# thu-ml/stochastic_gcn

Hardware: AMD Instinct MI355X
Metric: training edges/s (SpMM) (higher is better)
Workload: dtype f32

## Files before the change

### profiles/epoch_profile.py

```python
#!/usr/bin/env python
import glob
import os
import sqlite3
import sys

ROOT = os.path.dirname(os.path.dirname(os.path.abspath(__file__)))
sys.path.insert(0, ROOT)


def run(epochs):
    import torch
    import bench
    from stochastic_gcn_amd import _ffi
    for kv in os.environ.get("SGCN_TUNE", "").split():
        k, v = kv.split("=")
        _ffi.tune(k, int(v))
    from stochastic_gcn_amd import synthetic
    from stochastic_gcn_amd.flags import FLAGS
    over = {}
    for kv in os.environ.get("SGCN_FLAGS", "").split():
        k, v = kv.split("=")
        over[k] = type(getattr(FLAGS, k))(int(v)) if isinstance(getattr(FLAGS, k), (bool, int)) else float(v)
    if over:
        orig = FLAGS.update
        FLAGS.update = lambda **kw: (orig(**kw), orig(**over))[0]
    data = synthetic.reddit_like(seed=1, with_features=False)
    te = bench.train_epoch_leg(data, torch.device("cuda:0"), epochs=epochs)
    print(te, file=sys.stderr)


def summarize(src, steps):
    f = glob.glob(os.path.join(src, "**", "*results.db"), recursive=True)
    t = sqlite3.connect(f[0])
    rows = list(t.execute("select name,total_calls,total_duration,average,percentage from top_kernels"))
    tot = sum(r[2] for r in rows)
    print("== rocprofv3 --kernel-trace --stats of profiles/epoch_profile.py: %d training steps "
          "(batch 512, CVD+PP, S-Reddit), all kernels incl. set-up" % steps)
    print("GPU-busy total %.1f ms = %.3f ms per step (upper bound: includes the one-off PP SpMM and set-up kernels)"
          % (tot / 1e3, tot / 1e3 / steps))
    print("%-92s %8s %10s %12s %10s %6s" % ("kernel", "calls", "calls/step", "total_ms", "avg_us", "pct"))
    for r in rows[:40]:
        print("%-92s %8d %10.2f %12.1f %10.2f %6.2f" % (r[0][:92], r[1], r[1] / steps, r[2] / 1e3, r[3], r[4]))


if __name__ == "__main__" and not (len(sys.argv) > 1 and sys.argv[1] in ("--gaps", "--timeline", "--stepgaps")):
    if len(sys.argv) > 1 and sys.argv[1] == "--summarize":
        summarize(sys.argv[2], int(sys.argv[3]))
    else:
        run(int(sys.argv[1]) if len(sys.argv) > 1 else 3)


def gaps(src):
    f = glob.glob(os.path.join(src, "**", "*results.db"), recursive=True)
    t = sqlite3.connect(f[0])
    tabs = [r[0] for r in t.execute("select name from sqlite_master where type in ('table','view')")]
    view = "kernels" if "kernels" in tabs else None
    if view is None:
        print("tables:", tabs)
        return
    cols = [r[1] for r in t.execute("pragma table_info(%s)" % view)]
    rows = list(t.execute("select name, start, end from %s order by start" % view))
    import numpy as np
    st = np.array([r[1] for r in rows], dtype=np.int64)
    en = np.array([r[2] for r in rows], dtype=np.int64)
    names = [r[0] for r in rows]
    lo = len(rows) * 2 // 3
    gap = (st[lo + 1:] - en[lo:-1]) / 1e3
    dur = (en[lo:] - st[lo:]) / 1e3
    span = (en[-1] - st[lo]) / 1e3
    print("steady-state window: %d kernels over %.1f ms: busy %.1f ms (%.1f %%), idle between kernels %.1f ms"
          % (len(dur), span / 1e3, dur.sum() / 1e3, 100 * dur.sum() / span, gap.sum() / 1e3))
    print("gap between consecutive kernels: median %.2f us, mean %.2f us, p90 %.2f us, share of gaps > 4 us: %.1f %%"
          % (np.median(gap), gap.mean(), np.percentile(gap, 90), 100 * (gap > 4).mean()))
    adam = [i for i in range(lo, len(rows)) if "adam_" in names[i]]
    if len(adam) > 2:
        per = np.diff(st[adam]) / 1e3
        print("step period (adam to adam): median %.1f us; kernels per step %.1f"
              % (np.median(per), (adam[-1] - adam[0]) / (len(adam) - 1)))
    qcol = "queue_id" if "queue_id" in cols else ("stream_id" if "stream_id" in cols else None)
    if qcol and len(adam) > 2:
        qs = [r[0] for r in t.execute("select %s from %s order by start" % (qcol, view))]
        a, b = adam[0], adam[-1]
        nsteps = len(adam) - 1
        per_q = {}
        for i in range(a, b):
            k = per_q.setdefault(qs[i], [0, 0.0])
            k[0] += 1
            k[1] += (en[i] - st[i]) / 1e3
        for q, (cnt, us) in sorted(per_q.items(), key=lambda kv: -kv[1][1]):
            print("queue %s: %.1f kernels and %.1f us of kernel time per step" % (q, cnt / nsteps, us / nsteps))


if __name__ == "__main__" and len(sys.argv) > 1 and sys.argv[1] == "--gaps":
    gaps(sys.argv[2])


def timeline(src, n=70):
    f = glob.glob(os.path.join(src, "**", "*results.db"), recursive=True)
    t = sqlite3.connect(f[0])
    cols = [r[1] for r in t.execute("pragma table_info(kernels)")]
    qcol = "queue_id" if "queue_id" in cols else ("stream_id" if "stream_id" in cols else None)
    rows = list(t.execute("select name, start, end%s from kernels order by start" % ((", " + qcol) if qcol else "")))
    adam = [i for i, r in enumerate(rows) if "adam_" in r[0]]
    a, b = adam[len(adam) // 2], adam[len(adam) // 2 + 1]
    t0 = rows[a][2]
    print("columns:", cols)
    for r in rows[a:b + 1][:n]:
        print("%9.2f us  +%7.2f us  q=%s  %s" % ((r[1] - t0) / 1e3, (r[2] - r[1]) / 1e3, r[3] if qcol else "-", r[0][:70]))


if __name__ == "__main__" and len(sys.argv) > 1 and sys.argv[1] == "--timeline":
    timeline(sys.argv[2])


def stepgaps(src):
    import numpy as np
    f = glob.glob(os.path.join(src, "**", "*results.db"), recursive=True)
    t = sqlite3.connect(f[0])
    rows = list(t.execute("select name, start, end from kernels order by start"))
    adam = [i for i, r in enumerate(rows) if "adam_" in r[0]]
    adam = adam[len(adam) // 3:]
    lens = np.diff(adam)
    usual = int(np.bincount(lens).argmax())
    steps = [a for a, n in zip(adam[:-1], lens) if n == usual]
    gap = np.array([[rows[a + j + 1][1] - rows[a + j][2] for j in range(usual)] for a in steps]) / 1e3
    dur = np.array([[rows[a + j + 1][2] - rows[a + j + 1][1] for j in range(usual)] for a in steps]) / 1e3
    print("%d steady-state steps of %d kernels: idle in front of each kernel / its duration (median us; p90 of the idle)"
          % (len(steps), usual))
    for j in range(usual):
        print("  idle %6.2f (p90 %6.2f)  run %6.2f  %s" % (np.median(gap[:, j]), np.percentile(gap[:, j], 90),
                                                            np.median(dur[:, j]), rows[steps[0] + j + 1][0][:60]))
    print("  per step: idle %.1f us + kernels %.1f us" % (np.median(gap.sum(1)), np.median(dur.sum(1))))
    st = np.array([rows[a][1] for a in adam], dtype=np.int64)
    per = np.diff(st) / 1e3
    per = per[per < 2000]
    busy = np.array([sum(rows[i][2] - rows[i][1] for i in range(a + 1, b + 1)) for a, b in zip(adam[:-1], adam[1:])]) / 1e3
    busy = busy[:len(np.diff(st))][np.diff(st) / 1e3 < 2000]
    slow = [(int(i), round(float(p), 1)) for i, p in enumerate(np.diff(st) / 1e3) if 160 < p < 2000]
    print("  periods over 160 us (step index in the window, us):", slow[:40])
    print("  all %d steps: period mean %.1f / median %.1f / p90 %.1f / max %.1f us; kernel time mean %.1f / p90 %.1f us"
          % (len(per), per.mean(), np.median(per), np.percentile(per, 90), per.max(), busy.mean(), np.percentile(busy, 90)))


if __name__ == "__main__" and len(sys.argv) > 1 and sys.argv[1] == "--stepgaps":
    stepgaps(sys.argv[2])
```

### stochastic_gcn_amd/csrc/sgcn_agg.hip

```cpp
#include "sgcn_dev.h"
#include <type_traits>

namespace sgcn {

int group_lanes(int nvec);

template <class HT>
struct AggArgsT {
    const int32_t* a_rowptr; const int32_t* a_col; const float* a_val;
    const int32_t* f_rowptr; const int32_t* f_col; const float* f_val;
    const sgcn_seg_t* seg; int64_t nseg; int64_t nsegblk;
    const float* h; const float* mu; int64_t ldx;
    const HT* H; int64_t ldh;
    const int32_t* ifield; const int32_t* ffield; const float* s;
    float* out_h; float* out_mu; int64_t ldo;
    int32_t d, nvec, cvd, off, concat;
    float* ws; int64_t ldw;
    int32_t pchunks;
    float* accP_out; const float* accP_in;
};


template <int VW>
__device__ __forceinline__ void store_masked(float* p, typename Vec<VW>::type v, int left) {
    if (left >= VW) vstore<VW>(p, v);
    else vstore_head<VW>(p, v, left);
}

template <int G, int VW, class HT>
__device__ __forceinline__ void agg_apart(const AggArgsT<HT>& a, int row, int vi, int lig, bool act,
                                          typename Vec<VW>::type& acc1, typename Vec<VW>::type& acc2) {
    typedef typename Vec<VW>::type VT;
    acc1 = vzero<VW>(); acc2 = vzero<VW>();
    const int start = uniform_i<G>(a.a_rowptr[row]), end = uniform_i<G>(a.a_rowptr[row + 1]);
    const int64_t voff = (int64_t)vi * VW;
    for (int p0 = start; p0 < end; p0 += G) {
        const int n = min(G, end - p0);
        int mycol = 0, myhist = 0;
        float myval = 0.f;
        if (lig < n) {
            mycol = a.a_col[p0 + lig];
            myval = a.a_val[p0 + lig];
            myhist = a.ifield[mycol];
        }
        for (int j = 0; j < n; j++) {
            const int c = bcast_i<G>(mycol, j);
            const int hr = bcast_i<G>(myhist, j);
            const float v = bcast_f<G>(myval, j);
            if (!act) continue;
            const VT hb = hload<VW>(a.H + (int64_t)hr * a.ldh + voff);
            const VT xv = vload<VW>(a.h + (int64_t)c * a.ldx + voff);
            if constexpr (VW == 1 && !std::is_same<HT, float>::value) {
                if (a.cvd) {
                    const float mv = a.mu[(int64_t)c * a.ldx + voff];
                    acc1 = __builtin_fmaf(v, mv - hb, acc1);
                    acc2 = __builtin_fmaf(v, xv - mv, acc2);
                } else {
                    acc1 = __builtin_fmaf(v, xv, acc1);
                    acc2 = __builtin_fmaf(v, hb, acc2);
                }
            } else if (a.cvd) {
                const VT mv = vload<VW>(a.mu + (int64_t)c * a.ldx + voff);
                acc1 += v * (mv - hb);
                acc2 += v * (xv - mv);
            } else {
                acc1 += v * xv;
                acc2 += v * hb;
            }
        }
    }
}

template <int VW, class HT>
__device__ __forceinline__ void agg_epilogue(const AggArgsT<HT>& a, int row, int vi, bool act, typename Vec<VW>::type accP,
                                             typename Vec<VW>::type acc1, typename Vec<VW>::type acc2) {
    typedef typename Vec<VW>::type VT;
    if (!act) return;
    const int64_t voff = (int64_t)vi * VW;
    const int left = a.d - vi * VW;
    float* oh = a.out_h + (int64_t)row * a.ldo;
    if (a.cvd) {
        float* om = a.out_mu + (int64_t)row * a.ldo;
        const VT mu_nbr = acc1 + accP;
        const VT h_nbr = acc2 * a.s[row] + mu_nbr;
        store_masked<VW>(oh + a.off + voff, h_nbr, left);
        store_masked<VW>(om + a.off + voff, mu_nbr, left);
        if (a.concat) {
            store_masked<VW>(oh + voff, vload<VW>(a.h + (int64_t)row * a.ldx + voff), left);
            store_masked<VW>(om + voff, vload<VW>(a.mu + (int64_t)row * a.ldx + voff), left);
        }
    } else {
        const VT out = (acc1 - acc2) + accP;
        store_masked<VW>(oh + a.off + voff, out, left);
        if (a.concat) store_masked<VW>(oh + voff, vload<VW>(a.h + (int64_t)row * a.ldx + voff), left);
    }
}

template <int G, int VW, class HT>
__device__ __forceinline__ void agg_finish(const AggArgsT<HT>& a, int row, int vi, int lig, bool act,
                                           typename Vec<VW>::type accP) {
    typename Vec<VW>::type acc1, acc2;
    agg_apart<G, VW>(a, row, vi, lig, act, acc1, acc2);
    agg_epilogue<VW>(a, row, vi, act, accP, acc1, acc2);
}

static int p_chunks(int32_t d, const void* Hbar, int64_t ldh, const float* ws) {
    const int vw = pick_vw(d, {Hbar, ws}, {ldh, ((int64_t)d + 3) / 4 * 4});
    return kBlock / group_lanes((d + vw - 1) / vw) - 1;
}

constexpr int agg_max_chunks(int G, int VW) { return (kBlock / G) * (4 / VW) - 1 < 31 ? (kBlock / G) * (4 / VW) - 1 : 31; }

template <int G, int VW, int U, class HT>
__global__ __launch_bounds__(kBlock) void agg_row_kernel(AggArgsT<HT> a) {
    typedef typename Vec<VW>::type VT;
    constexpr int NG = kBlock / G, NP = NG - 1;
    constexpr int NC = agg_max_chunks(G, VW);
    __shared__ float part[NC + 2][G * VW];
    const int lig = threadIdx.x & (G - 1), gq = threadIdx.x / G;
    const int slab = (int)(blockIdx.x / a.nseg);
    const int64_t s = blockIdx.x % a.nseg;
    int row, start, end, slot;
    if (a.seg) {
        const sgcn_seg_t sg = a.seg[s];
        row = sg.row; start = sg.start; end = sg.end; slot = sg.slot;
    } else {
        row = (int)s; start = a.f_rowptr[s]; end = a.f_rowptr[s + 1]; slot = -1;
    }
    row = uniform_i<G>(row); start = uniform_i<G>(start);
    end = uniform_i<G>(end); slot = uniform_i<G>(slot);
    const int vi = slab * G + lig;
    const bool act = vi < a.nvec;
    const bool finish_here = slot < 0 && !a.accP_out;
    const HT* Hl = a.H + (int64_t)vi * VW;

    const int nc = a.pchunks;
    if (gq < NP) {
        const int chunk = (end - start + nc - 1) / nc;
        for (int ck = gq; ck < nc; ck += NP) {
            const int gs = start + ck * chunk, ge = min(end, gs + chunk);
            VT accP = vzero<VW>();
            for (int p0 = gs; p0 < ge; p0 += G) {
                const int n = min(G, ge - p0);
                int myrow = 0;
                float myval = 0.f;
                if (lig < n) {
                    myrow = a.ffield[a.f_col[p0 + lig]];
                    myval = a.f_val[p0 + lig];
                }
                hpin<HT, VW>(myrow); hpin<HT, VW>(myval);
                for (int j = 0; j < n; j += U) {
                    typename HRaw<HT, VW>::type b[U];
                    float v[U];
#pragma unroll
                    for (int u = 0; u < U; u++) {
                        const bool in = j + u < n;
                        const int c = bcast_i<G>(myrow, in ? j + u : 0);
                        v[u] = in ? bcast_f<G>(myval, j + u) : 0.f;
                        b[u] = (act && in) ? hraw<VW>(Hl + (int64_t)c * a.ldh) : hraw_zero<HT, VW>();
                    }
#pragma unroll
                    for (int u = 0; u < U; u++) { hpin<HT, VW>(b[u]); accP += v[u] * hwiden<VW>(b[u]); }
                }
            }
            vstore<VW>(&part[ck][lig * VW], accP);
        }
    } else if (finish_here) {
        VT acc1, acc2;
        agg_apart<G, VW>(a, row, vi, lig, act, acc1, acc2);
        vstore<VW>(&part[NC][lig * VW], acc1);
        vstore<VW>(&part[NC + 1][lig * VW], acc2);
    }
    __syncthreads();
    if (gq != 0) return;
    VT accP = vload<VW>(&part[0][lig * VW]);
    if (nc == NP) {
#pragma unroll
        for (int q = 1; q < NP; q++) accP += vload<VW>(&part[q][lig * VW]);
    } else {
        for (int q = 1; q < nc; q++) accP += vload<VW>(&part[q][lig * VW]);
    }
    if (slot >= 0) { if (act) vstore<VW>(a.ws + (int64_t)slot * a.ldw + (int64_t)vi * VW, accP); }
    else if (a.accP_out) { if (act) vstore<VW>(a.accP_out + (int64_t)row * a.ldw + (int64_t)vi * VW, accP); }
    else agg_epilogue<VW>(a, row, vi, act, accP, vload<VW>(&part[NC][lig * VW]), vload<VW>(&part[NC + 1][lig * VW]));
}

template <int G, int VW, class HT>
__global__ __launch_bounds__(kBlock) void agg_fix_kernel(AggArgsT<HT> a, const sgcn_fix_t* fix, int64_t nfix) {
    typedef typename Vec<VW>::type VT;
    constexpr int GPB = kBlock / G;
    const int lig = threadIdx.x & (G - 1);
    const int64_t nfblk = (nfix + GPB - 1) / GPB;
    const int slab = (int)(blockIdx.x / nfblk);
    const int64_t f = (blockIdx.x % nfblk) * GPB + threadIdx.x / G;
    if (f >= nfix) return;
    const sgcn_fix_t fx = fix[f];
    const int vi = slab * G + lig;
    const bool act = vi < a.nvec;
    VT accP = vzero<VW>();
    if (act) {
        const float* w = a.ws + (int64_t)fx.first_slot * a.ldw + (int64_t)vi * VW;
        for (int q = 0; q < fx.nslots; q++) accP += vload<VW>(w + (int64_t)q * a.ldw);
    }
    if (a.accP_out) { if (act) vstore<VW>(a.accP_out + (int64_t)fx.row * a.ldw + (int64_t)vi * VW, accP); }
    else agg_finish<G, VW>(a, uniform_i<G>(fx.row), vi, lig, act, accP);
}

template <int G, int VW, class HT>
__global__ __launch_bounds__(kBlock) void agg_post_kernel(AggArgsT<HT> a, int32_t n1) {
    typedef typename Vec<VW>::type VT;
    constexpr int GPB = kBlock / G;
    const int lig = threadIdx.x & (G - 1);
    const int64_t nrblk = ((int64_t)n1 + GPB - 1) / GPB;
    const int slab = (int)(blockIdx.x / nrblk);
    const int64_t row = (blockIdx.x % nrblk) * GPB + threadIdx.x / G;
    if (row >= n1) return;
    const int vi = slab * G + lig;
    const bool act = vi < a.nvec;
    const VT accP = act ? vload<VW>(a.accP_in + row * a.ldw + (int64_t)vi * VW) : vzero<VW>();
    agg_finish<G, VW>(a, uniform_i<G>((int)row), vi, lig, act, accP);
}

template <int VW, class HT>
static int launch_agg_post(int G, const AggArgsT<HT>& a, int32_t n1, hipStream_t st) {
    const int nslab = (a.nvec + G - 1) / G;
#define SGCN_AGGP_CASE(GG)                                                                               \
    case GG: {                                                                                           \
        const int64_t nrblk = ((int64_t)n1 + (kBlock / GG) - 1) / (kBlock / GG);                          \
        hipLaunchKernelGGL((agg_post_kernel<GG, VW, HT>), dim3((unsigned)(nrblk * nslab)), dim3(kBlock), 0, st, a, n1); \
        break;                                                                                           \
    }
    switch (G) {
        SGCN_AGGP_CASE(8)
        SGCN_AGGP_CASE(16)
        SGCN_AGGP_CASE(32)
        SGCN_AGGP_CASE(64)
        default: return fail(SGCN_ERR_INVALID, "vr_aggregate_post: bad group %d", G);
    }
#undef SGCN_AGGP_CASE
    SGCN_HIP_TRY(hipGetLastError());
    return SGCN_OK;
}

template <int VW, class HT>
static int launch_agg(int G, const AggArgsT<HT>& a, const sgcn_plan_t* plan, hipStream_t st) {
    const int nslab = (a.nvec + G - 1) / G;
    SGCN_REQUIRE(a.pchunks >= 1 && a.pchunks <= agg_max_chunks(G, VW), "vr_aggregate: %d chunks of a P row, at most %d here",
                 a.pchunks, agg_max_chunks(G, VW));
    const int64_t nblocks = a.nseg * nslab;
    SGCN_REQUIRE(nblocks < (1ll << 31), "vr_aggregate: grid too large");
#define SGCN_AGG_CASE(GG)                                                                          \
    case GG: {                                                                                     \
        hipLaunchKernelGGL((agg_row_kernel<GG, VW, 16, HT>), dim3((unsigned)nblocks), dim3(kBlock), 0,  \
                           st, a);                                                                 \
        if (plan && plan->nfix > 0) {                                                              \
            const int64_t nfblk = (plan->nfix + (kBlock / GG) - 1) / (kBlock / GG);               \
            hipLaunchKernelGGL((agg_fix_kernel<GG, VW, HT>), dim3((unsigned)(nfblk * nslab)),          \
                               dim3(kBlock), 0, st, a, plan->dev_fix, plan->nfix);                 \
        }                                                                                          \
        break;                                                                                     \
    }
    switch (G) {
        SGCN_AGG_CASE(8)
        SGCN_AGG_CASE(16)
        SGCN_AGG_CASE(32)
        SGCN_AGG_CASE(64)
        default: return fail(SGCN_ERR_INVALID, "vr_aggregate: bad group %d", G);
    }
#undef SGCN_AGG_CASE
    SGCN_HIP_TRY(hipGetLastError());
    return SGCN_OK;
}

}

using namespace sgcn;

template <class HT>
static const void* vw_table(const HT* Hbar) { return std::is_same<HT, float>::value ? Hbar : nullptr; }

template <class HT>
static int vr_aggregate(const char* who, const int32_t* a_rowptr, const int32_t* a_col, const float* a_val,
                        const int32_t* f_rowptr, const int32_t* f_col, const float* f_val, int32_t n1, int32_t n0, int32_t nf,
                        int32_t d, const float* h, const float* mu, int64_t ldx, const HT* Hbar, int64_t ldh,
                        const int32_t* ifield, const int32_t* ffield, const float* s, float* out_h, float* out_mu, int64_t ldo,
                        int32_t cvd, int32_t concat_self, const sgcn_plan_t* f_plan, void* stream) {
    constexpr bool kH16 = !std::is_same<HT, float>::value;
    SGCN_REQUIRE(n1 >= 0 && n0 >= 0 && nf >= 0 && d >= 0, "%s: negative size", who);
    if constexpr (kH16) { if (int rc = h16_table_ok(who, Hbar, ldh, d)) return rc; }
    if (n1 == 0 || d == 0) return SGCN_OK;
    SGCN_REQUIRE(a_rowptr && f_rowptr && h && Hbar && ifield && out_h, "%s: null operand", who);
    SGCN_REQUIRE(nf == 0 || ffield, "%s: null ffield", who);
    SGCN_REQUIRE(!cvd || (mu && s && out_mu), "%s: cvd needs mu, s, out_mu", who);
    SGCN_REQUIRE(n1 <= n0 || !concat_self, "%s: concat_self needs n1 <= n0", who);
    const int64_t width = concat_self ? 2 * (int64_t)d : d;
    SGCN_REQUIRE(ldx >= d && ldh >= d && ldo >= width, "%s: leading dimension too small", who);

    AggArgsT<HT> a{};
    a.a_rowptr = a_rowptr; a.a_col = a_col; a.a_val = a_val;
    a.f_rowptr = f_rowptr; a.f_col = f_col; a.f_val = f_val;
    a.h = h; a.mu = mu; a.ldx = ldx; a.H = Hbar; a.ldh = ldh;
    a.ifield = ifield; a.ffield = ffield; a.s = s;
    a.out_h = out_h; a.out_mu = out_mu; a.ldo = ldo;
    a.d = d; a.cvd = cvd; a.concat = concat_self; a.off = concat_self ? d : 0;
    a.nseg = n1;
    if (f_plan) {
        SGCN_REQUIRE(f_plan->dev_seg && f_plan->nseg >= n1, "%s: malformed plan", who);
        a.seg = f_plan->dev_seg; a.nseg = f_plan->nseg;
        a.ws = f_plan->dev_ws; a.ldw = ((int64_t)d + 3) / 4 * 4;
        if (f_plan->nfix > 0) {
            SGCN_REQUIRE(f_plan->dev_fix && f_plan->dev_ws, "%s: plan needs dev_fix/dev_ws", who);
            SGCN_REQUIRE(f_plan->ws_elems >= f_plan->nslots * a.ldw, "%s: workspace too small", who);
        }
    }
    int vw = pick_vw(d, {h, mu, vw_table(Hbar), out_h, out_mu, f_plan ? f_plan->dev_ws : nullptr}, {ldx, ldh, ldo});
    if (concat_self) while (vw > 1 && d % vw != 0) vw >>= 1;
    a.nvec = (d + vw - 1) / vw;
    const int G = group_lanes(a.nvec);
    a.pchunks = p_chunks(d, vw_table(Hbar), ldh, f_plan ? f_plan->dev_ws : nullptr);
    a.nsegblk = (a.nseg + (kBlock / G) - 1) / (kBlock / G);
    hipStream_t st = (hipStream_t)stream;
    if (vw == 4) return launch_agg<4>(G, a, f_plan, st);
    if (vw == 2) return launch_agg<2>(G, a, f_plan, st);
    return launch_agg<1>(G, a, f_plan, st);
}

template <class HT>
static int vr_aggregate_pre(const char* who, const int32_t* f_rowptr, const int32_t* f_col, const float* f_val, int32_t n1,
                            int32_t nf, int32_t d, const HT* Hbar, int64_t ldh, const int32_t* ffield, float* accP,
                            const sgcn_plan_t* f_plan, void* stream) {
    constexpr bool kH16 = !std::is_same<HT, float>::value;
    SGCN_REQUIRE(n1 >= 0 && nf >= 0 && d >= 0, "%s: negative size", who);
    if constexpr (kH16) { if (int rc = h16_table_ok(who, Hbar, ldh, d)) return rc; }
    if (n1 == 0 || d == 0) return SGCN_OK;
    SGCN_REQUIRE(f_rowptr && Hbar && accP && ldh >= d, "%s: bad operand", who);
    SGCN_REQUIRE(nf == 0 || ffield, "%s: null ffield", who);
    AggArgsT<HT> a{};
    a.f_rowptr = f_rowptr; a.f_col = f_col; a.f_val = f_val;
    a.H = Hbar; a.ldh = ldh; a.ffield = ffield; a.d = d;
    a.ldw = ((int64_t)d + 3) / 4 * 4;
    a.accP_out = accP;
    a.nseg = n1;
    if (f_plan) {
        SGCN_REQUIRE(f_plan->dev_seg && f_plan->nseg >= n1, "%s: malformed plan", who);
        a.seg = f_plan->dev_seg; a.nseg = f_plan->nseg; a.ws = f_plan->dev_ws;
        if (f_plan->nfix > 0) {
            SGCN_REQUIRE(f_plan->dev_fix && f_plan->dev_ws, "%s: plan needs dev_fix/dev_ws", who);
            SGCN_REQUIRE(f_plan->ws_elems >= f_plan->nslots * a.ldw, "%s: workspace too small", who);
        }
    }
    const int vw = pick_vw(d, {vw_table(Hbar), accP, f_plan ? f_plan->dev_ws : nullptr}, {ldh, a.ldw});
    a.nvec = (d + vw - 1) / vw;
    const int G = group_lanes(a.nvec);
    a.pchunks = p_chunks(d, vw_table(Hbar), ldh, f_plan ? f_plan->dev_ws : nullptr);
    a.nsegblk = (a.nseg + (kBlock / G) - 1) / (kBlock / G);
    hipStream_t st = (hipStream_t)stream;
    if (vw == 4) return launch_agg<4>(G, a, f_plan, st);
    if (vw == 2) return launch_agg<2>(G, a, f_plan, st);
    return launch_agg<1>(G, a, f_plan, st);
}

template <class HT>
static int vr_aggregate_post(const char* who, const int32_t* a_rowptr, const int32_t* a_col, const float* a_val, int32_t n1,
                             int32_t n0, int32_t d, const float* h, const float* mu, int64_t ldx, const HT* Hbar, int64_t ldh,
                             const int32_t* ifield, const float* s, float* out_h, float* out_mu, int64_t ldo, int32_t cvd,
                             int32_t concat_self, const float* accP, void* stream) {
    constexpr bool kH16 = !std::is_same<HT, float>::value;
    SGCN_REQUIRE(n1 >= 0 && n0 >= 0 && d >= 0, "%s: negative size", who);
    if constexpr (kH16) { if (int rc = h16_table_ok(who, Hbar, ldh, d)) return rc; }
    if (n1 == 0 || d == 0) return SGCN_OK;
    SGCN_REQUIRE(a_rowptr && h && Hbar && ifield && out_h && accP, "%s: null operand", who);
    SGCN_REQUIRE(!cvd || (mu && s && out_mu), "%s: cvd needs mu, s, out_mu", who);
    SGCN_REQUIRE(n1 <= n0 || !concat_self, "%s: concat_self needs n1 <= n0", who);
    const int64_t width = concat_self ? 2 * (int64_t)d : d;
    SGCN_REQUIRE(ldx >= d && ldh >= d && ldo >= width, "%s: leading dimension too small", who);
    AggArgsT<HT> a{};
    a.a_rowptr = a_rowptr; a.a_col = a_col; a.a_val = a_val;
    a.h = h; a.mu = mu; a.ldx = ldx; a.H = Hbar; a.ldh = ldh; a.ifield = ifield; a.s = s;
    a.out_h = out_h; a.out_mu = out_mu; a.ldo = ldo;
    a.d = d; a.cvd = cvd; a.concat = concat_self; a.off = concat_self ? d : 0;
    a.ldw = ((int64_t)d + 3) / 4 * 4;
    a.accP_in = accP;
    int vw = pick_vw(d, {h, mu, vw_table(Hbar), out_h, out_mu, accP}, {ldx, ldh, ldo, a.ldw});
    if (concat_self) while (vw > 1 && d % vw != 0) vw >>= 1;
    a.nvec = (d + vw - 1) / vw;
    const int G = group_lanes(a.nvec);
    hipStream_t st = (hipStream_t)stream;
    if (vw == 4) return launch_agg_post<4>(G, a, n1, st);
    if (vw == 2) return launch_agg_post<2>(G, a, n1, st);
    return launch_agg_post<1>(G, a, n1, st);
}

extern "C" int sgcn_vr_aggregate_f32(const int32_t* a_rowptr, const int32_t* a_col, const float* a_val,
                                     const int32_t* f_rowptr, const int32_t* f_col, const float* f_val, int32_t n1,
                                     int32_t n0, int32_t nf, int32_t d, const float* h, const float* mu, int64_t ldx,
                                     const float* Hbar, int64_t ldh, const int32_t* ifield, const int32_t* ffield,
                                     const float* s, float* out_h, float* out_mu, int64_t ldo, int32_t cvd,
                                     int32_t concat_self, const sgcn_plan_t* f_plan, void* stream) {
    return vr_aggregate<float>("vr_aggregate", a_rowptr, a_col, a_val, f_rowptr, f_col, f_val, n1, n0, nf, d, h, mu, ldx, Hbar,
                               ldh, ifield, ffield, s, out_h, out_mu, ldo, cvd, concat_self, f_plan, stream);
}

extern "C" int sgcn_vr_aggregate_pre_f32(const int32_t* f_rowptr, const int32_t* f_col, const float* f_val, int32_t n1,
                                         int32_t nf, int32_t d, const float* Hbar, int64_t ldh, const int32_t* ffield,
                                         float* accP, const sgcn_plan_t* f_plan, void* stream) {
    return vr_aggregate_pre<float>("vr_aggregate_pre", f_rowptr, f_col, f_val, n1, nf, d, Hbar, ldh, ffield, accP, f_plan, stream);
}

extern "C" int sgcn_vr_aggregate_post_f32(const int32_t* a_rowptr, const int32_t* a_col, const float* a_val, int32_t n1,
                                          int32_t n0, int32_t d, const float* h, const float* mu, int64_t ldx,
                                          const float* Hbar, int64_t ldh, const int32_t* ifield, const float* s,
                                          float* out_h, float* out_mu, int64_t ldo, int32_t cvd, int32_t concat_self,
                                          const float* accP, void* stream) {
    return vr_aggregate_post<float>("vr_aggregate_post", a_rowptr, a_col, a_val, n1, n0, d, h, mu, ldx, Hbar, ldh, ifield, s,
                                    out_h, out_mu, ldo, cvd, concat_self, accP, stream);
}

extern "C" int sgcn_vr_aggregate_h16(const int32_t* a_rowptr, const int32_t* a_col, const float* a_val,
                                     const int32_t* f_rowptr, const int32_t* f_col, const float* f_val, int32_t n1,
                                     int32_t n0, int32_t nf, int32_t d, const float* h, const float* mu, int64_t ldx,
                                     const uint16_t* Hbar, int64_t ldh, const int32_t* ifield, const int32_t* ffield,
                                     const float* s, float* out_h, float* out_mu, int64_t ldo, int32_t cvd,
                                     int32_t concat_self, const sgcn_plan_t* f_plan, void* stream) {
    return vr_aggregate<uint16_t>("vr_aggregate_h16", a_rowptr, a_col, a_val, f_rowptr, f_col, f_val, n1, n0, nf, d, h, mu, ldx,
                                  Hbar, ldh, ifield, ffield, s, out_h, out_mu, ldo, cvd, concat_self, f_plan, stream);
}

extern "C" int sgcn_vr_aggregate_pre_h16(const int32_t* f_rowptr, const int32_t* f_col, const float* f_val, int32_t n1,
                                         int32_t nf, int32_t d, const uint16_t* Hbar, int64_t ldh, const int32_t* ffield,
                                         float* accP, const sgcn_plan_t* f_plan, void* stream) {
    return vr_aggregate_pre<uint16_t>("vr_aggregate_pre_h16", f_rowptr, f_col, f_val, n1, nf, d, Hbar, ldh, ffield, accP, f_plan,
                                      stream);
}

extern "C" int sgcn_vr_aggregate_post_h16(const int32_t* a_rowptr, const int32_t* a_col, const float* a_val, int32_t n1,
                                          int32_t n0, int32_t d, const float* h, const float* mu, int64_t ldx,
                                          const uint16_t* Hbar, int64_t ldh, const int32_t* ifield, const float* s,
                                          float* out_h, float* out_mu, int64_t ldo, int32_t cvd, int32_t concat_self,
                                          const float* accP, void* stream) {
    return vr_aggregate_post<uint16_t>("vr_aggregate_post_h16", a_rowptr, a_col, a_val, n1, n0, d, h, mu, ldx, Hbar, ldh, ifield,
                                       s, out_h, out_mu, ldo, cvd, concat_self, accP, stream);
}
```

Baseline: 7.402 billion.

## Stash split-row partials in output and batch slot sums in fix kernel

Result: no change. 7.400 billion (-0.0%).

```diff
diff --git a/profiles/epoch_profile.py b/profiles/epoch_profile.py
--- a/profiles/epoch_profile.py
+++ b/profiles/epoch_profile.py
@@ -43,7 +43,7 @@
         print("%-92s %8d %10.2f %12.1f %10.2f %6.2f" % (r[0][:92], r[1], r[1] / steps, r[2] / 1e3, r[3], r[4]))
 
 
-if __name__ == "__main__" and not (len(sys.argv) > 1 and sys.argv[1] in ("--gaps", "--timeline", "--stepgaps")):
+if __name__ == "__main__" and not (len(sys.argv) > 1 and sys.argv[1] in ("--gaps", "--timeline", "--stepgaps", "--kernels")):
     if len(sys.argv) > 1 and sys.argv[1] == "--summarize":
         summarize(sys.argv[2], int(sys.argv[3]))
     else:
@@ -144,3 +144,36 @@
 
 if __name__ == "__main__" and len(sys.argv) > 1 and sys.argv[1] == "--stepgaps":
     stepgaps(sys.argv[2])
+
+
+def kernel_table(src):
+    import numpy as np
+    f = glob.glob(os.path.join(src, "**", "*results.db"), recursive=True)
+    t = sqlite3.connect(f[0])
+    rows = list(t.execute("select name, start, end from kernels order by start"))
+    adam = [i for i, r in enumerate(rows) if "adam_" in r[0]]
+    a, b = adam[len(adam) // 3], adam[-1]
+    steps = len(adam) - 1 - len(adam) // 3
+    dur = {}
+    for name, st, en in rows[a + 1:b + 1]:
+        dur.setdefault(name, []).append((en - st) / 1e3)
+    print("== rocprofv3 --kernel-trace of profiles/epoch_profile.py: %d steady-state training steps (batch 512, CVD+PP, "
+          "S-Reddit; evaluation sweeps between the epochs included)" % steps)
+    print("%-80s %8s %10s %9s %9s %9s" % ("kernel", "calls", "calls/step", "mean_us", "p50_us", "p90_us"))
+    for name, d in sorted(dur.items(), key=lambda kv: -sum(kv[1])):
+        d = np.array(d)
+        print("%-80s %8d %10.2f %9.2f %9.2f %9.2f" % (name[:80], d.size, d.size / steps, d.mean(), np.median(d),
+                                                      np.percentile(d, 90)))
+    dur = {}
+    for name, st, en in rows[b + 1:]:
+        dur.setdefault(name, []).append((en - st) / 1e3)
+    print("== behind the last training step (validation sweeps): the ten kernels with the most time")
+    print("%-80s %8s %10s %9s %9s %9s" % ("kernel", "calls", "total_ms", "mean_us", "p50_us", "p90_us"))
+    for name, d in sorted(dur.items(), key=lambda kv: -sum(kv[1]))[:10]:
+        d = np.array(d)
+        print("%-80s %8d %10.3f %9.2f %9.2f %9.2f" % (name[:80], d.size, d.sum() / 1e3, d.mean(), np.median(d),
+                                                      np.percentile(d, 90)))
+
+
+if __name__ == "__main__" and len(sys.argv) > 1 and sys.argv[1] == "--kernels":
+    kernel_table(sys.argv[2])
diff --git a/stochastic_gcn_amd/csrc/sgcn_agg.hip b/stochastic_gcn_amd/csrc/sgcn_agg.hip
--- a/stochastic_gcn_amd/csrc/sgcn_agg.hip
+++ b/stochastic_gcn_amd/csrc/sgcn_agg.hip
@@ -25,6 +25,20 @@
 __device__ __forceinline__ void store_masked(float* p, typename Vec<VW>::type v, int left) {
     if (left >= VW) vstore<VW>(p, v);
     else vstore_head<VW>(p, v, left);
+}
+
+template <int VW>
+__device__ __forceinline__ typename Vec<VW>::type load_masked(const float* p, int left) {
+    if (left >= VW) return vload<VW>(p);
+    typename Vec<VW>::type v = vzero<VW>();
+    if constexpr (VW > 1) {
+        float t[VW];
+#pragma unroll
+        for (int e = 0; e < VW; e++) t[e] = p[min(e, left - 1)];
+#pragma unroll
+        for (int e = 0; e < VW; e++) v[e] = e < left ? t[e] : 0.f;
+    }
+    return v;
 }
 
 template <int G, int VW, class HT>
@@ -71,9 +85,26 @@
     }
 }
 
+template <int VW>
+struct AggSelf { float s; typename Vec<VW>::type h, mu; };
+
+template <int VW, class HT>
+__device__ __forceinline__ AggSelf<VW> agg_self(const AggArgsT<HT>& a, int row, int vi, bool act) {
+    AggSelf<VW> x;
+    x.s = 0.f; x.h = vzero<VW>(); x.mu = vzero<VW>();
+    if (!act) return x;
+    const int64_t voff = (int64_t)vi * VW;
+    if (a.cvd) x.s = a.s[row];
+    if (a.concat) {
+        x.h = vload<VW>(a.h + (int64_t)row * a.ldx + voff);
+        if (a.cvd) x.mu = vload<VW>(a.mu + (int64_t)row * a.ldx + voff);
+    }
+    return x;
+}
+
 template <int VW, class HT>
 __device__ __forceinline__ void agg_epilogue(const AggArgsT<HT>& a, int row, int vi, bool act, typename Vec<VW>::type accP,
-                                             typename Vec<VW>::type acc1, typename Vec<VW>::type acc2) {
+                                             typename Vec<VW>::type acc1, typename Vec<VW>::type acc2, const AggSelf<VW>& x) {
     typedef typename Vec<VW>::type VT;
     if (!act) return;
     const int64_t voff = (int64_t)vi * VW;
@@ -82,18 +113,74 @@
     if (a.cvd) {
         float* om = a.out_mu + (int64_t)row * a.ldo;
         const VT mu_nbr = acc1 + accP;
-        const VT h_nbr = acc2 * a.s[row] + mu_nbr;
+        const VT h_nbr = acc2 * x.s + mu_nbr;
         store_masked<VW>(oh + a.off + voff, h_nbr, left);
         store_masked<VW>(om + a.off + voff, mu_nbr, left);
         if (a.concat) {
-            store_masked<VW>(oh + voff, vload<VW>(a.h + (int64_t)row * a.ldx + voff), left);
-            store_masked<VW>(om + voff, vload<VW>(a.mu + (int64_t)row * a.ldx + voff), left);
+            store_masked<VW>(oh + voff, x.h, left);
+            store_masked<VW>(om + voff, x.mu, left);
         }
     } else {
         const VT out = (acc1 - acc2) + accP;
         store_masked<VW>(oh + a.off + voff, out, left);
-        if (a.concat) store_masked<VW>(oh + voff, vload<VW>(a.h + (int64_t)row * a.ldx + voff), left);
-    }
+        if (a.concat) store_masked<VW>(oh + voff, x.h, left);
+    }
+}
+
+template <int VW, class HT>
+__device__ __forceinline__ void agg_epilogue(const AggArgsT<HT>& a, int row, int vi, bool act, typename Vec<VW>::type accP,
+                                             typename Vec<VW>::type acc1, typename Vec<VW>::type acc2) {
+    agg_epilogue<VW>(a, row, vi, act, accP, acc1, acc2, agg_self<VW>(a, row, vi, act));
+}
+
+template <int VW, class HT>
+__device__ __forceinline__ void agg_stash(const AggArgsT<HT>& a, int row, int vi, bool act, typename Vec<VW>::type acc1,
+                                          typename Vec<VW>::type acc2) {
+    if (!act) return;
+    const int64_t at = (int64_t)row * a.ldo + a.off + (int64_t)vi * VW;
+    const int left = a.d - vi * VW;
+    if (a.cvd) {
+        store_masked<VW>(a.out_mu + at, acc1, left);
+        store_masked<VW>(a.out_h + at, acc2, left);
+    } else {
+        store_masked<VW>(a.out_h + at, acc1 - acc2, left);
+    }
+}
+
+template <int VW, class HT>
+__device__ __forceinline__ void agg_unstash(const AggArgsT<HT>& a, int row, int vi, bool act, typename Vec<VW>::type& acc1,
+                                            typename Vec<VW>::type& acc2) {
+    acc1 = vzero<VW>(); acc2 = vzero<VW>();
+    if (!act) return;
+    const int64_t at = (int64_t)row * a.ldo + a.off + (int64_t)vi * VW;
+    const int left = a.d - vi * VW;
+    if (a.cvd) {
+        acc1 = load_masked<VW>(a.out_mu + at, left);
+        acc2 = load_masked<VW>(a.out_h + at, left);
+    } else {
+        acc1 = load_masked<VW>(a.out_h + at, left);
+    }
+}
+
+constexpr int kSlotBatch = 8;
+
+template <int VW>
+__device__ __forceinline__ typename Vec<VW>::type agg_slot_batch(const float* w, int q0, int nslots, int64_t ldw,
+                                                                  typename Vec<VW>::type acc) {
+    typename Vec<VW>::type b[kSlotBatch];
+#pragma unroll
+    for (int u = 0; u < kSlotBatch; u++) b[u] = vload<VW>(w + (int64_t)min(q0 + u, nslots - 1) * ldw);
+#pragma unroll
+    for (int u = 0; u < kSlotBatch; u++) acc += q0 + u < nslots ? b[u] : vzero<VW>();
+    return acc;
+}
+
+template <int VW>
+__device__ __forceinline__ typename Vec<VW>::type agg_slot_sum(const float* w, int nslots, int64_t ldw) {
+    typename Vec<VW>::type acc = vzero<VW>();
+    if (nslots <= kSlotBatch) return agg_slot_batch<VW>(w, 0, nslots, ldw, acc);
+    for (int q0 = 0; q0 < nslots; q0 += kSlotBatch) acc = agg_slot_batch<VW>(w, q0, nslots, ldw, acc);
+    return acc;
 }
 
 template <int G, int VW, class HT>
@@ -131,7 +218,6 @@
     end = uniform_i<G>(end); slot = uniform_i<G>(slot);
     const int vi = slab * G + lig;
     const bool act = vi < a.nvec;
-    const bool finish_here = slot < 0 && !a.accP_out;
     const HT* Hl = a.H + (int64_t)vi * VW;
 
     const int nc = a.pchunks;
@@ -148,7 +234,7 @@
                     myrow = a.ffield[a.f_col[p0 + lig]];
                     myval = a.f_val[p0 + lig];
                 }
-                hpin<HT, VW>(myrow); hpin<HT, VW>(myval);
+                if constexpr (VW > 1) asm volatile("" : "+v"(myrow), "+v"(myval));
                 for (int j = 0; j < n; j += U) {
                     typename HRaw<HT, VW>::type b[U];
                     float v[U];
@@ -165,11 +251,15 @@
             }
             vstore<VW>(&part[ck][lig * VW], accP);
         }
-    } else if (finish_here) {
+    } else if (!a.accP_out && (slot < 0 || start == uniform_i<G>(a.f_rowptr[row]))) {
         VT acc1, acc2;
         agg_apart<G, VW>(a, row, vi, lig, act, acc1, acc2);
-        vstore<VW>(&part[NC][lig * VW], acc1);
-        vstore<VW>(&part[NC + 1][lig * VW], acc2);
+        if (slot < 0) {
+            vstore<VW>(&part[NC][lig * VW], acc1);
+            vstore<VW>(&part[NC + 1][lig * VW], acc2);
+        } else {
+            agg_stash<VW>(a, row, vi, act, acc1, acc2);
+        }
     }
     __syncthreads();
     if (gq != 0) return;
@@ -185,25 +275,37 @@
     else agg_epilogue<VW>(a, row, vi, act, accP, vload<VW>(&part[NC][lig * VW]), vload<VW>(&part[NC + 1][lig * VW]));
 }
 
+template <int VW, bool CVD, bool CONCAT, class HT>
+__device__ __forceinline__ void agg_fix_row(AggArgsT<HT> a, int row, int vi, const float* w, int nslots) {
+    typedef typename Vec<VW>::type VT;
+    a.cvd = CVD; a.concat = CONCAT;
+    VT acc1, acc2;
+    agg_unstash<VW>(a, row, vi, true, acc1, acc2);
+    const AggSelf<VW> x = agg_self<VW>(a, row, vi, true);
+    const VT accP = agg_slot_sum<VW>(w, nslots, a.ldw);
+    agg_epilogue<VW>(a, row, vi, true, accP, acc1, acc2, x);
+}
+
 template <int G, int VW, class HT>
 __global__ __launch_bounds__(kBlock) void agg_fix_kernel(AggArgsT<HT> a, const sgcn_fix_t* fix, int64_t nfix) {
-    typedef typename Vec<VW>::type VT;
     constexpr int GPB = kBlock / G;
     const int lig = threadIdx.x & (G - 1);
     const int64_t nfblk = (nfix + GPB - 1) / GPB;
     const int slab = (int)(blockIdx.x / nfblk);
     const int64_t f = (blockIdx.x % nfblk) * GPB + threadIdx.x / G;
-    if (f >= nfix) return;
+    const int vi = slab * G + lig;
+    if (f >= nfix || vi >= a.nvec) return;
     const sgcn_fix_t fx = fix[f];
-    const int vi = slab * G + lig;
-    const bool act = vi < a.nvec;
-    VT accP = vzero<VW>();
-    if (act) {
-        const float* w = a.ws + (int64_t)fx.first_slot * a.ldw + (int64_t)vi * VW;
-        for (int q = 0; q < fx.nslots; q++) accP += vload<VW>(w + (int64_t)q * a.ldw);
-    }
-    if (a.accP_out) { if (act) vstore<VW>(a.accP_out + (int64_t)fx.row * a.ldw + (int64_t)vi * VW, accP); }
-    else agg_finish<G, VW>(a, uniform_i<G>(fx.row), vi, lig, act, accP);
+    const float* w = a.ws + (int64_t)fx.first_slot * a.ldw + (int64_t)vi * VW;
+    if (a.accP_out) {
+        vstore<VW>(a.accP_out + (int64_t)fx.row * a.ldw + (int64_t)vi * VW, agg_slot_sum<VW>(w, fx.nslots, a.ldw));
+    } else if (a.cvd) {
+        if (a.concat) agg_fix_row<VW, true, true>(a, fx.row, vi, w, fx.nslots);
+        else agg_fix_row<VW, true, false>(a, fx.row, vi, w, fx.nslots);
+    } else {
+        if (a.concat) agg_fix_row<VW, false, true>(a, fx.row, vi, w, fx.nslots);
+        else agg_fix_row<VW, false, false>(a, fx.row, vi, w, fx.nslots);
+    }
 }
 
 template <int G, int VW, class HT>
```
